# AIS-Bonn/stillleben

Measured on AMD Instinct MI355X. Metric: scenes/sec (settle + 640x480 6-ch GT render), 20-obj YCB-like, higher is better.
Workload: dtype f32; 1 GPU; C2: 20 of 21 procedural YCB-like objects (8k verts/16k tris, 1024^2 texture each) per scene; per step and GPU 32768 scenes are staged (random stack), settled (100 frames x 4 substeps), framed (camera, light, shadow matrix) and rendered at 640x480 (rgb, coord+depth, class, instance, normals; shadows on, SSAO on) -- all four stages inside the timed region; render_chunk=512, objects=20, settle_streams=1, render_streams=2, pair_contact_budget=0, parallelism=1 GPU

## Files before the change

include/slhip.h:

```cpp
#ifndef SLHIP_H
#define SLHIP_H

#include <stdint.h>

#ifdef __cplusplus
extern "C" {
#endif

#define SLHIP_ABI_VERSION 5
#define SLHIP_NUM_LIGHTS 3


typedef struct {
    float* d_env;
    float* d_irradiance;
    float* d_prefilter;
    float* d_brdf_lut;
    uint32_t env_size, env_levels;
    uint32_t irr_size;
    uint32_t pre_size, pre_levels;
    uint32_t lut_size;
} slhip_light_map;

typedef struct {
// ... 252 lines not shown
    uint32_t max_contacts_per_scene;
    uint32_t pair_contact_budget;
    uint32_t resume;
    uint32_t max_body_pairs_per_scene;
    float stabilization_threshold;
    uint32_t _pad_params;
} slhip_settle_params;
#define SLHIP_STAB_DAMPING          0.5f
#define SLHIP_STAB_GRAVITY          0.9f
#define SLHIP_STAB_FREEZE_INTERVAL  1.5f
#define SLHIP_STAB_FREEZE_TOLERANCE 0.25f
#define SLHIP_STAB_MAX_INTERACTIONS 10

#define SLHIP_MAX_BODIES     400
#define SLHIP_DEFAULT_HULL_PAIRS 2048
#define SLHIP_DEFAULT_CONTACTS   1024
#define SLHIP_PAIR_CACHE_DENSE_HULLS 256

int slhip_settle(const slhip_settle_scene* d_scenes, uint32_t n_scenes,
                 slhip_body* d_bodies, const slhip_hull* d_hulls, const float* d_hull_verts,
                 const slhip_settle_params* params, void* d_scratch, uint64_t scratch_bytes,
                 void* stream);
#define SLHIP_SETTLE_REFUSED_BODIES 1u
#define SLHIP_SETTLE_REFUSED_HULLS  2u
int slhip_settle_caps(const void* d_scratch, uint32_t n_scenes, const slhip_settle_params* params,
                      uint64_t counts[10], void* stream);
int slhip_settle_status(const void* d_scratch, uint32_t n_scenes, uint32_t* h_status, uint32_t* h_n_refused,
                        void* stream);
int slhip_settle_timing_enable(int on);
int slhip_settle_timings(float avg_ms_out[5], uint32_t launches_out[5]);
int slhip_settle_timing_every(uint32_t every);
int slhip_settle_timings_by_step(float* ms_out, uint32_t* steps_out, uint32_t capacity, uint32_t* n_out);
int slhip_settle_solver_wave_lds(void);
int slhip_settle_scratch_bytes(uint32_t n_scenes, const slhip_settle_params* params, uint64_t* bytes_out);

int slhip_overlap_any(const slhip_settle_scene* d_scenes, uint32_t n_scenes,
                      const slhip_body* d_bodies, const slhip_hull* d_hulls,
                      const float* d_hull_verts, uint8_t* d_flags, void* stream);


int slhip_diff_sobel_valid(const int16_t* d_inst, const float* d_depth, int depth_stride, int H, int W,
                           uint8_t* d_valid, void* stream);

int slhip_diff_dilate(const uint8_t* d_mask, const uint8_t* d_valid, const float* d_coords, int coord_stride,
                      int H, int W, uint8_t* d_out_mask, float* d_out_coords, void* stream);

int slhip_diff_image_gradients(const uint8_t* d_rgb, const uint8_t* d_valid, int H, int W, float* d_grad_x,
                               float* d_grad_y, void* stream);

int slhip_diff_pose_backward(const uint8_t* d_rgb, const float* d_coord, const int16_t* d_inst,
                             const float* d_grad_img, const float* h_proj, const float* d_poses,
                             const int32_t* d_obj_inst, int n_obj, int H, int W, uint8_t* d_valid,
                             double* d_acc, float* d_out, void* stream);
int slhip_diff_pose_backward_batch(const uint8_t* d_rgb, const float* d_coord, const int16_t* d_inst,
                                   const float* d_grad_img, uint64_t grad_stride_floats, const float* h_proj,
                                   const float* d_poses, const int32_t* d_obj_inst, int n_obj, int n_hyp, int H, int W,
                                   uint8_t* d_valid, double* d_acc, float* d_out, void* stream);

int slhip_light_map_floats(uint32_t env_size, uint32_t env_levels, uint32_t irr_size, uint32_t pre_size,
                           uint32_t pre_levels, uint32_t lut_size, uint64_t out[4]);
int slhip_light_map_build(const float* d_equirect, int H, int W, const slhip_light_map* lm, void* stream);

typedef struct {
    float translation[6];
    float scaling[3];
    float blur_kernel[25];
// ... 173 lines not shown
```

stillleben_amd/_abi.py:

```python
import ctypes as C
import os

import numpy as np

NUM_LIGHTS = 3
CHUNK_TRIS = 256

DRAW_HAS_BASE_TEX = 1
DRAW_VERTEX_COLORS = 2
DRAW_CASTS_SHADOW = 4
DRAW_ALPHA_TEST = 8
DRAW_NO_VERTEX_ID = 16
DRAW_HAS_NORMAL_TEX = 32
DRAW_HAS_MR_TEX = 64
DRAW_HAS_OCCLUSION_TEX = 128
DRAW_HAS_EMISSIVE_TEX = 256
DRAW_HAS_STICKER = 512
SAMPLER_DEFAULT = 0x10 | 0x20 | (2 << 6)

OUT_RGB = 0x01
OUT_COORD = 0x02
OUT_CLASS = 0x04
OUT_INSTANCE = 0x08
OUT_NORMALS = 0x10
# ... 276 lines not shown
    L.slhip_diff_sobel_valid.argtypes = [C.c_void_p, C.c_void_p, C.c_int, C.c_int, C.c_int, C.c_void_p, C.c_void_p]
    L.slhip_diff_dilate.argtypes = [C.c_void_p, C.c_void_p, C.c_void_p, C.c_int, C.c_int, C.c_int, C.c_void_p, C.c_void_p, C.c_void_p]
    L.slhip_diff_image_gradients.argtypes = [C.c_void_p, C.c_void_p, C.c_int, C.c_int, C.c_void_p, C.c_void_p, C.c_void_p]
    L.slhip_diff_pose_backward.argtypes = [C.c_void_p] * 7 + [C.c_int, C.c_int, C.c_int] + [C.c_void_p] * 4
    L.slhip_diff_pose_backward_batch.argtypes = [C.c_void_p] * 4 + [C.c_uint64] + [C.c_void_p] * 3 + [C.c_int] * 4 + [C.c_void_p] * 4
    L.slhip_diff_vertex_backward.argtypes = [C.c_void_p] * 8 + [C.c_int, C.c_int, C.c_int] + [C.c_void_p] * 4
    L.slhip_settle.argtypes = [C.c_void_p, C.c_uint32, C.c_void_p, C.c_void_p, C.c_void_p, C.c_void_p,
                               C.c_void_p, C.c_uint64, C.c_void_p]
    L.slhip_settle_status.argtypes = [C.c_void_p, C.c_uint32, C.c_void_p, C.POINTER(C.c_uint32), C.c_void_p]
    L.slhip_host_shadow_matrices.argtypes = [C.c_void_p, C.c_void_p, C.c_void_p]
    L.slhip_host_normal_matrix.argtypes = [C.c_void_p, C.c_void_p]
    L.slhip_host_convex_hull.argtypes = [C.c_void_p, C.c_uint32, C.c_void_p, C.c_uint32, C.POINTER(C.c_uint32)]
    L.slhip_host_fill_holes.argtypes = [C.c_void_p, C.c_uint32, C.c_uint32, C.c_uint32]
    L.slhip_records_count.argtypes = [C.c_void_p, C.c_uint32, C.c_void_p, C.c_void_p, C.POINTER(C.c_uint32), C.POINTER(C.c_uint32)]
    L.slhip_records_build_render.argtypes = [C.c_void_p, C.c_uint32, C.c_void_p, C.c_void_p, C.c_uint32, C.c_void_p, C.c_void_p,
                                             C.c_uint32, C.c_void_p, C.c_uint32]
    L.slhip_render_object_stats.argtypes = [
        C.POINTER(MeshPool), C.c_void_p, C.c_void_p, C.c_void_p, C.c_uint32, C.c_uint32, C.c_uint32, C.c_uint32, C.c_uint32,
        C.POINTER(RenderScratch), C.c_uint32, C.c_void_p, C.c_uint64, C.c_void_p, C.POINTER(C.c_uint64), C.c_void_p,
    ]
    L.slhip_render_object_stats_bytes.argtypes = [C.c_uint32, C.c_uint32, C.c_uint32, C.c_uint32, C.POINTER(C.c_uint64)]
    L.slhip_render_object_masks.argtypes = [
        C.POINTER(MeshPool), C.c_void_p, C.c_void_p, C.c_void_p, C.c_uint32, C.c_uint32, C.c_uint32, C.c_uint32, C.c_uint32,
        C.POINTER(RenderScratch), C.c_uint32, C.c_void_p, C.c_uint64, C.c_void_p, C.POINTER(C.c_uint64),
        C.c_void_p, C.c_void_p, C.c_uint64, C.POINTER(C.c_uint64), C.c_void_p,
    ]
    L.slhip_render_object_masks_bytes.argtypes = [C.c_uint32, C.c_uint32, C.c_uint32, C.c_uint32, C.POINTER(C.c_uint64),
                                                  C.POINTER(C.c_uint64)]
    L.slhip_object_masks_expand.argtypes = [C.c_void_p, C.c_void_p, C.c_uint32, C.c_uint32, C.c_uint32, C.c_uint32, C.c_uint32,
                                            C.c_void_p, C.c_uint64, C.c_void_p, C.c_void_p]
    L.slhip_render_ssao_skipped.argtypes = [C.c_void_p, C.c_uint32, C.c_uint32, C.c_uint32, C.POINTER(C.c_uint64 * 2), C.c_void_p]
    L.slhip_render_ssao_levels.argtypes = [C.c_void_p, C.c_uint32, C.c_uint32, C.c_uint32, C.POINTER(C.c_uint64 * 8), C.c_void_p]
    L.slhip_render_ssao_level_tables.argtypes = [C.POINTER(C.c_float * 5), C.POINTER(C.c_uint32 * 6), C.POINTER(C.c_uint8 * 384)]
    L.slhip_settle_caps.argtypes = [C.c_void_p, C.c_uint32, C.c_void_p, C.POINTER(C.c_uint64 * 10), C.c_void_p]
    L.slhip_settle_timing_enable.argtypes = [C.c_int]
    L.slhip_settle_timings.argtypes = [C.POINTER(C.c_float * 5), C.POINTER(C.c_uint32 * 5)]
    if hasattr(L, "slhip_settle_timing_every"):
        L.slhip_settle_timing_every.argtypes = [C.c_uint32]
        L.slhip_settle_timings_by_step.argtypes = [C.c_void_p, C.c_void_p, C.c_uint32, C.POINTER(C.c_uint32)]
    L.slhip_settle_scratch_bytes.argtypes = [C.c_uint32, C.c_void_p, C.POINTER(C.c_uint64)]
    L.slhip_overlap_any.argtypes = [C.c_void_p, C.c_uint32, C.c_void_p, C.c_void_p, C.c_void_p, C.c_void_p, C.c_void_p]
    L.slhip_light_map_floats.argtypes = [C.c_uint32] * 6 + [C.POINTER(C.c_uint64 * 4)]
    L.slhip_light_map_build.argtypes = [C.c_void_p, C.c_int, C.c_int, C.c_void_p, C.c_void_p]
    L.slhip_camera_model.argtypes = [C.c_void_p, C.c_void_p, C.c_void_p, C.c_uint32, C.c_int, C.c_int, C.c_void_p, C.c_void_p]
    L.slhip_stream_create_cu_range.argtypes = [C.c_uint32, C.c_uint32, C.POINTER(C.c_void_p)]
    L.slhip_stream_destroy.argtypes = [C.c_void_p]
    L.slhip_synth_stage.argtypes = [C.c_void_p] * 8
    L.slhip_synth_place.argtypes = [C.c_void_p] * 10
    if hasattr(L, "slhip_synth_place_env"):
        L.slhip_synth_place_env.argtypes = [C.c_void_p, C.POINTER(SynthEnv)] + [C.c_void_p] * 10
    if hasattr(L, "slhip_synth_place_view"):
        L.slhip_synth_place_view.argtypes = [C.c_void_p, C.POINTER(SynthEnv), C.POINTER(SynthView)] + [C.c_void_p] * 10
    L.slhip_comm_unique_id.argtypes = [C.c_void_p]
    L.slhip_comm_create.argtypes = [C.c_void_p, C.c_int, C.c_int, C.POINTER(C.c_void_p)]
    L.slhip_comm_destroy.argtypes = [C.c_void_p]
    L.slhip_comm_info.argtypes = [C.c_void_p, C.POINTER(C.c_int), C.POINTER(C.c_int)]
    L.slhip_allgather.argtypes = [C.c_void_p, C.c_void_p, C.c_void_p, C.c_uint64, C.c_void_p]
    L.slhip_allgather_group.argtypes = [C.c_void_p, C.c_uint32, C.c_void_p, C.c_void_p, C.c_void_p, C.c_void_p]
    _LIB = L
    return L


def check(status, what):
    if status != 0:
        msg = lib().slhip_last_error()
        raise SlhipError("%s failed (%d): %s" % (what, status, msg.decode() if msg else "?"))
# ... 1 lines not shown
```

stillleben_amd/csrc/slhip_settle.hip:

```cpp
#include "slhip_common.h"
#include <vector>
#include <cstdlib>

namespace {

static_assert(sizeof(slhip_body) == 304, "slhip_body layout");
static_assert(sizeof(slhip_hull) == 64, "slhip_hull layout");
static_assert(sizeof(slhip_settle_params) == 128, "slhip_settle_params layout");

constexpr int kMaxContactsPerHP = 4;
constexpr float kInf = 3.0e38f;
constexpr float kDepthWeight = 30.0f;

struct v3 { float x, y, z; };
struct quat { float x, y, z, w; };
struct m3 { float m[9]; };

__device__ __forceinline__ v3 V(float x, float y, float z) { v3 r; r.x = x; r.y = y; r.z = z; return r; }
__device__ __forceinline__ v3 add(v3 a, v3 b) { return V(a.x + b.x, a.y + b.y, a.z + b.z); }
__device__ __forceinline__ v3 sub(v3 a, v3 b) { return V(a.x - b.x, a.y - b.y, a.z - b.z); }
__device__ __forceinline__ v3 scale(v3 a, float s) { return V(a.x * s, a.y * s, a.z * s); }
__device__ __forceinline__ v3 neg(v3 a) { return V(-a.x, -a.y, -a.z); }
__device__ __forceinline__ float dot(v3 a, v3 b) { return fmaf(a.z, b.z, fmaf(a.y, b.y, a.x * b.x)); }
__device__ __forceinline__ v3 cross(v3 a, v3 b)
{
    return V(a.y * b.z - a.z * b.y, a.z * b.x - a.x * b.z, a.x * b.y - a.y * b.x);
}
__device__ __forceinline__ v3 madd(v3 a, v3 b, float s)
{
    return V(fmaf(b.x, s, a.x), fmaf(b.y, s, a.y), fmaf(b.z, s, a.z));
}
__device__ __forceinline__ v3 m3_mul(const m3& M, v3 v)
{
// ... 1409 lines not shown
    for (auto& r : g_settle_timing.pending) {
        float ms = 0.0f;
        if (failed || hipEventSynchronize(r.e1) != hipSuccess || hipEventElapsedTime(&ms, r.e0, r.e1) != hipSuccess) { failed = true; continue; }
        acc[r.kernel] += ms;
        ++n[r.kernel];
        if (by_step_ms) {
            if (r.kernel == 0) {
                row_open = rows < cap;
                if (row_open) { if (steps_out) steps_out[rows] = r.step; ++rows; }
            }
            if (row_open) by_step_ms[5 * (size_t)(rows - 1) + r.kernel] = ms;
        }
    }
    for (hipEvent_t e : g_settle_timing.events) (void)hipEventDestroy(e);
    g_settle_timing.events.clear();
    g_settle_timing.pending.clear();
    if (n_out) *n_out = rows;
    if (failed) {
        slhip::set_error("slhip_settle_timings: event readback failed");
        return -1;
    }
    for (int k = 0; k < 5; ++k) {
        if (avg_ms_out) avg_ms_out[k] = n[k] ? (float)(acc[k] / n[k]) : 0.0f;
        if (launches_out) launches_out[k] = n[k];
    }
    return 0;
}

extern "C" int slhip_settle_timings(float avg_ms_out[5], uint32_t launches_out[5])
{
    return settle_timings_read(avg_ms_out, launches_out, nullptr, nullptr, 0, nullptr);
}

#ifdef SLHIP_ROW_PROFILE
extern "C" int slhip_settle_row_profile(unsigned long long out[8])
{
    SLHIP_CHECK(hipDeviceSynchronize());
    SLHIP_CHECK(hipMemcpyFromSymbol(out, HIP_SYMBOL(g_row_prof), 8 * sizeof(unsigned long long)));
    unsigned long long zero[8] = {0, 0, 0, 0, 0, 0, 0, 0};
    SLHIP_CHECK(hipMemcpyToSymbol(HIP_SYMBOL(g_row_prof), zero, sizeof(zero)));
    return 0;
}
#endif

static int g_last_solve_lds = 0;
extern "C" int slhip_settle_solver_wave_lds(void) { return g_last_solve_lds; }

extern "C" int slhip_settle_timing_every(uint32_t every)
{
    g_settle_timing_every = every ? every : 1u;
    return 0;
}

extern "C" int slhip_settle_timings_by_step(float* ms_out, uint32_t* steps_out, uint32_t capacity, uint32_t* n_out)
{
    if (!ms_out || !n_out) {
        slhip::set_error("slhip_settle_timings_by_step: null output");
        return -1;
    }
    return settle_timings_read(nullptr, nullptr, ms_out, steps_out, capacity, n_out);
}

extern "C" int slhip_settle_scratch_bytes(uint32_t n_scenes, const slhip_settle_params* params, uint64_t* bytes_out)
{
    if (!bytes_out) {
        slhip::set_error("slhip_settle_scratch_bytes: null output");
        return -1;
    }
    *bytes_out = settle_scratch_bytes(n_scenes, params);
    return 0;
}

extern "C" int slhip_settle(const slhip_settle_scene* d_scenes, uint32_t n_scenes, slhip_body* d_bodies,
                            const slhip_hull* d_hulls, const float* d_hull_verts, const slhip_settle_params* params,
                            void* d_scratch, uint64_t scratch_bytes, void* stream_)
{
// ... 8 lines not shown
        return -1;
    }
    const SettleDims D = settle_dims(params);
    const int nb_cap = D.nb_cap;
    if (nb_cap > SLHIP_MAX_BODIES) {
        slhip::set_error("slhip_settle: at most %d bodies per scene", SLHIP_MAX_BODIES);
        return -1;
    }
    {
        if (n_scenes > 65535u) {
            slhip::set_error("slhip_settle: at most 65535 scenes per launch");
            return -1;
        }
        ProfScratch* prof_w = reinterpret_cast<ProfScratch*>(d_scratch);
        DriveAcc* drive_w = reinterpret_cast<DriveAcc*>(prof_w + n_scenes);
        char* base = reinterpret_cast<char*>(d_scratch) + settle_fixed_bytes(n_scenes, D);
        PairCache pc;
        pc.base = reinterpret_cast<int4*>(base);
        pc.stride = D.cache_stride;
        pc.hashed = D.cache_hashed;
        WideBufs W = wide_carve(base + settle_cache_bytes(n_scenes, D), n_scenes, nb_cap, D.lh_cap, D.p_cap, D.c_cap, D.bp_cap);
        if (((uint64_t)n_scenes << W.pair_bits) > (1ull << 32)) {
            slhip::set_error("slhip_settle: n_scenes x max_hull_pairs_per_scene exceeds the 32-bit work list entries");
            return -1;
        }
        const BeginLds BL = begin_layout(nb_cap, D.lh_cap);
        const FinishLds FL = finish_layout(nb_cap, W.g_cap);
        int solve_lds = 20 * 1024;
        if (solve_min_lds(nb_cap, W.g_cap) > solve_lds) solve_lds = (solve_min_lds(nb_cap, W.g_cap) + 1023) & ~1023;
        if (const char* e = getenv("SLHIP_SOLVE_LDS_KB")) { const int kb = atoi(e) * 1024; if (kb >= solve_min_lds(nb_cap, W.g_cap) && kb <= 160 * 1024) solve_lds = kb; }
        int max_class = 2;
        if (const char* e = getenv("SLHIP_SOLVE_SPW")) { const int v = atoi(e); max_class = v == 1 ? 0 : v == 2 ? 1 : 2; }
        W.solve_lds = solve_lds; W.solve_max_class = max_class;
        g_last_solve_lds = solve_lds;
        if (BL.total > 160 * 1024 || FL.total > 160 * 1024 || solve_lds > 160 * 1024) {
            slhip::set_error("slhip_settle: scenes of %d bodies / %d hulls do not fit the kernels' LDS", nb_cap, D.lh_cap);
            return -1;
        }
        SLHIP_CHECK(hipFuncSetAttribute(reinterpret_cast<const void*>(k_w_begin), hipFuncAttributeMaxDynamicSharedMemorySize, BL.total));
        SLHIP_CHECK(hipFuncSetAttribute(reinterpret_cast<const void*>(k_w_finish), hipFuncAttributeMaxDynamicSharedMemorySize, FL.total));
        SLHIP_CHECK(hipFuncSetAttribute(reinterpret_cast<const void*>(k_w_solve), hipFuncAttributeMaxDynamicSharedMemorySize, solve_lds));
        if (params->resume == 0u) k_w_prologue<<<n_scenes, 64, 0, stream>>>(d_scenes, d_bodies, d_hulls, W, prof_w, pc);
        const unsigned list_stride = n_scenes * (unsigned)D.p_cap;
        unsigned work_grid = n_scenes < 16u ? n_scenes * 8u : n_scenes;
        if (const char* e = getenv("SLHIP_WORK_GRID_DIV")) { const unsigned d = (unsigned)atoi(e); if (d > 1u && work_grid / d >= 64u) work_grid /= d; }
        bool persistent = n_scenes <= kPersistentMaxScenes;
        if (const char* e = getenv("SLHIP_SETTLE_PERSISTENT")) persistent = atoi(e) != 0;
        if (persistent) {
            WideBufs Wp = W;
            Wp.solve_lds = max(solve_lds, 32 * 1024);
            const int lds = max(max(BL.total, FL.total), Wp.solve_lds);
            SLHIP_CHECK(hipFuncSetAttribute(reinterpret_cast<const void*>(k_w_persistent), hipFuncAttributeMaxDynamicSharedMemorySize, lds));
            unsigned grid = n_scenes < 4096u ? n_scenes : 4096u;
            if (const char* e = getenv("SLHIP_SETTLE_PERSISTENT_GRID")) { const unsigned g = (unsigned)atoi(e); if (g > 0u && g < grid) grid = g; }
            k_w_persistent<<<grid, 64, lds, stream>>>(d_scenes, d_bodies, d_hulls, d_hull_verts, *params, Wp, BL, FL, pc, drive_w, list_stride, n_scenes);
            SLHIP_LAUNCH_CHECK();
            return 0;
        }
        uint32_t lockstep_frames = params->frames;
        if (const char* e = getenv("SLHIP_SETTLE_SWITCH_FRAME")) { const int v = atoi(e); if (v >= 0 && (uint32_t)v < params->frames) lockstep_frames = (uint32_t)v; }
        uint32_t step = params->resume;
        for (uint32_t f = 0; f < lockstep_frames; ++f)
            for (uint32_t sub = 0; sub < params->substeps; ++sub, ++step) {
                constexpr size_t kMaxTimedEvents = 1u << 16;
                bool timed = g_settle_timing.on && step % g_settle_timing_every == 0u && g_settle_timing.events.size() < kMaxTimedEvents;
                hipEvent_t ev[6];
// ... 112 lines not shown
```

stillleben_amd/csrc/slhip_settle_wide.inc:

```

struct WideHdr {
    int n_hp, n_groups, n_plane_groups, n_active, n_active_before_pairs, ncol, status, n_hulls;
    int hp_overflow, hp_found;
    int g_overflow;
    int lds_need, lds_class;
};
struct PlanePM { int stamp, count, c_off, id[4], pad; };
static_assert(sizeof(PlanePM) == 32, "PlanePM layout");

__device__ __forceinline__ int cache_x(int seed_n, bool has, unsigned step) { return (seed_n & 3) | ((has ? 1 : 0) << 2) | (int)(step << 3); }
__device__ __forceinline__ int sv_pack(int idx) { return (idx & 0xff) | ((idx >> 16) << 8); }
__device__ __forceinline__ int sv_unpack(int c) { return (c & 0xff) | (((c >> 8) & 0xff) << 16); }

enum { kCapSpillSteps = 0, kCapContactDropSteps, kCapPairDropSteps, kCapMaxContacts, kCapMaxPairs, kCapReducedSteps, kCapGroupDropSteps, kCapContactSum, kCapWords = 8 };
constexpr unsigned short kCulled = 0xffff;

__device__ const float kNoImpulse[4] = {0.0f, 0.0f, 0.0f, 0.0f};

struct WideBufs {
    WideHdr* hdr;
    WBody* wb;
    HullRef* lh;
    int* body_lh;
    HullPair* hp;
    unsigned short* hp_off;
    unsigned short* hp_grp;
    MainResult* mr;
    StagePt* stage;
    Contact* ac;
    Group* groups;
    unsigned short* order;
    unsigned* lpt_count;
    unsigned short* lpt_table;
    unsigned* work;
    PM* pm;
    float* lnout;
    PlanePM* pp;
    unsigned* caps;
    unsigned* work_count;
    int nb_cap, lh_cap;
    int p_cap, c_cap;
    int g_cap, o_stride;
    int pair_bits;
    int solve_lds;
    int solve_max_class;
};
constexpr int kLptWords = 3 * 256 + 3 * 8;

__host__ __device__ inline size_t wide_align(size_t x) { return (x + 255u) & ~(size_t)255u; }

__host__ __device__ inline int wide_g_cap(int nb_cap, int p_cap, int bp_cap)
{
    long long pairs = (long long)nb_cap * (nb_cap - 1) / 2;
    if (pairs > p_cap) pairs = p_cap;
    const long long lim = bp_cap > 0 ? (long long)bp_cap : 12ll * nb_cap + 64;
    if (pairs > lim) pairs = lim;
    return nb_cap + (int)pairs;
}

inline uint64_t wide_bytes(uint32_t n, int nb_cap, int lh_cap, int p_cap, int c_cap, int bp_cap)
{
    const size_t g_cap = (size_t)wide_g_cap(nb_cap, p_cap, bp_cap), o_stride = 2 * g_cap + 66;
    uint64_t b = 0;
    b += wide_align((size_t)n * sizeof(WideHdr));
    b += wide_align((size_t)n * nb_cap * sizeof(WBody));
    b += wide_align((size_t)n * lh_cap * sizeof(HullRef));
    b += wide_align((size_t)n * (nb_cap + 1) * sizeof(int));
    b += wide_align((size_t)n * p_cap * sizeof(HullPair));
    b += wide_align((size_t)n * (p_cap + 1) * sizeof(unsigned short));
    b += wide_align((size_t)n * p_cap * sizeof(unsigned short));
    b += wide_align((size_t)n * p_cap * sizeof(MainResult));
    b += wide_align((size_t)n * p_cap * 4 * sizeof(StagePt));
    b += wide_align((size_t)n * c_cap * sizeof(Contact));
    b += wide_align((size_t)n * g_cap * sizeof(Group));
    b += wide_align((size_t)n * o_stride * sizeof(unsigned short));
    b += wide_align((size_t)5 * n * p_cap * sizeof(unsigned));
    b += wide_align((size_t)2 * n * p_cap * sizeof(PM));
    b += wide_align((size_t)n * c_cap * sizeof(float));
// ... 4 lines not shown
    b += wide_align((size_t)3 * 256 * ((n + 7u) / 8u) * sizeof(unsigned short));
    return b;
}

inline WideBufs wide_carve(char* base, uint32_t n, int nb_cap, int lh_cap, int p_cap, int c_cap, int bp_cap)
{
    WideBufs B;
    B.nb_cap = nb_cap; B.lh_cap = lh_cap; B.p_cap = p_cap; B.c_cap = c_cap;
    B.g_cap = wide_g_cap(nb_cap, p_cap, bp_cap); B.o_stride = 2 * B.g_cap + 66;
    B.pair_bits = 1;
    while ((1 << B.pair_bits) < p_cap) ++B.pair_bits;
    char* p = base;
    auto take = [&](size_t bytes) { char* r = p; p += wide_align(bytes); return r; };
    B.hdr = reinterpret_cast<WideHdr*>(take((size_t)n * sizeof(WideHdr)));
    B.wb = reinterpret_cast<WBody*>(take((size_t)n * nb_cap * sizeof(WBody)));
    B.lh = reinterpret_cast<HullRef*>(take((size_t)n * lh_cap * sizeof(HullRef)));
    B.body_lh = reinterpret_cast<int*>(take((size_t)n * (nb_cap + 1) * sizeof(int)));
    B.hp = reinterpret_cast<HullPair*>(take((size_t)n * p_cap * sizeof(HullPair)));
    B.hp_off = reinterpret_cast<unsigned short*>(take((size_t)n * (p_cap + 1) * sizeof(unsigned short)));
    B.hp_grp = reinterpret_cast<unsigned short*>(take((size_t)n * p_cap * sizeof(unsigned short)));
    B.mr = reinterpret_cast<MainResult*>(take((size_t)n * p_cap * sizeof(MainResult)));
    B.stage = reinterpret_cast<StagePt*>(take((size_t)n * p_cap * 4 * sizeof(StagePt)));
    B.ac = reinterpret_cast<Contact*>(take((size_t)n * c_cap * sizeof(Contact)));
    B.groups = reinterpret_cast<Group*>(take((size_t)n * B.g_cap * sizeof(Group)));
    B.order = reinterpret_cast<unsigned short*>(take((size_t)n * B.o_stride * sizeof(unsigned short)));
    B.work = reinterpret_cast<unsigned*>(take((size_t)5 * n * p_cap * sizeof(unsigned)));
    B.pm = reinterpret_cast<PM*>(take((size_t)2 * n * p_cap * sizeof(PM)));
    B.lnout = reinterpret_cast<float*>(take((size_t)n * c_cap * sizeof(float)));
    B.pp = reinterpret_cast<PlanePM*>(take((size_t)n * nb_cap * sizeof(PlanePM)));
    B.caps = reinterpret_cast<unsigned*>(take((size_t)n * kCapWords * sizeof(unsigned)));
    B.work_count = reinterpret_cast<unsigned*>(take(64));
    B.lpt_count = reinterpret_cast<unsigned*>(take(kLptWords * sizeof(unsigned)));
    B.lpt_table = reinterpret_cast<unsigned short*>(take((size_t)3 * 256 * ((n + 7u) / 8u) * sizeof(unsigned short)));
    B.solve_lds = 0; B.solve_max_class = 2;
    return B;
}

struct PairCache {
    int4* base;
    unsigned stride;
    int hashed;
};
__device__ __forceinline__ int4* pair_cache_slot(const PairCache& pc, int s, int n_hulls, int la, int lb, unsigned parity, bool claim)
{
    int4* tab = pc.base + (size_t)s * pc.stride;
    if (!pc.hashed) {
        if (n_hulls <= 0 || (unsigned)n_hulls * (unsigned)n_hulls > pc.stride) return nullptr;
        return tab + (size_t)la * n_hulls + lb;
    }
    const unsigned half = pc.stride >> 1, mask = half - 1u;
    tab += (size_t)(parity & 1u) * half;
    const unsigned key = ((unsigned)la | ((unsigned)lb << 16)) + 1u;
    unsigned h = (key * 2654435761u) >> 7;
    for (unsigned probe = 0; probe < half; ++probe, ++h) {
        int4* e = tab + (h & mask);
        unsigned k = (unsigned)e->w;
        if (k == 0u) {
            if (!claim) return nullptr;
            k = atomicCAS(reinterpret_cast<unsigned*>(&e->w), 0u, key);
            if (k == 0u) k = key;
        }
        if (k == key) return e;
    }
    return nullptr;
}

__device__ __forceinline__ void lanes_copy(void* dst, const void* src, int bytes, int hl, int n_lanes)
// ... 59 lines not shown
        if (lane == 0) { prof_all[s].status = SLHIP_SETTLE_REFUSED_HULLS; H->status = 1; }
        return;
    }
    if (lane == 0) {
        body_lh[nb] = n_lh;
        prof_all[s].status = 0;
        H->status = 0;
        H->n_hp = 0; H->n_groups = 0; H->n_plane_groups = 0; H->n_active = 0; H->n_active_before_pairs = 0; H->ncol = 0;
        H->n_hulls = n_lh;
    }
    {
        const unsigned n = pc.hashed ? pc.stride : (unsigned)(n_lh * n_lh);
        if (n <= pc.stride) {
            int4* z = pc.base + (size_t)s * pc.stride;
            for (unsigned k = lane; k < n; k += 64) z[k] = make_int4(0, 0, 0, 0);
        }
    }
}

struct BeginLds { int off_wb, off_lh, off_body_lh, off_band, off_plist, total; };
__host__ __device__ inline BeginLds begin_layout(int nb_cap, int lh_cap)
{
    BeginLds L;
    int o = 0;
    auto take = [&](int bytes) { const int r = o; o += (bytes + 15) & ~15; return r; };
    L.off_wb = take(nb_cap * (int)sizeof(WBody));
    L.off_lh = take(lh_cap * (int)sizeof(HullRef));
    L.off_body_lh = take((nb_cap + 1) * 4);
    L.off_band = take(4 * kBandCap * (int)sizeof(BandPt));
    L.off_plist = take(64);
    L.total = o;
    return L;
}

template <bool kFileWork>
__device__ __forceinline__ void begin_scene(char* smem, const int s, const unsigned n_scenes, const slhip_settle_scene* __restrict__ scenes,
                                            slhip_body* bodies_all, const slhip_hull* __restrict__ hulls, const float* __restrict__ hull_verts,
                                            const slhip_settle_params& prm, const WideBufs& W, const BeginLds& L, DriveAcc* drive_all, unsigned step)
{
    const int lane = threadIdx.x;
    WideHdr* H = W.hdr + s;
    if (H->status != 0) return;
    WBody* wb = reinterpret_cast<WBody*>(smem + L.off_wb);
    HullRef* lh = reinterpret_cast<HullRef*>(smem + L.off_lh);
    int* body_lh = reinterpret_cast<int*>(smem + L.off_body_lh);
    BandPt* band = reinterpret_cast<BandPt*>(smem + L.off_band);
    unsigned char* plist = reinterpret_cast<unsigned char*>(smem + L.off_plist);
    const float4* gv = reinterpret_cast<const float4*>(hull_verts);
    const f3* hv = reinterpret_cast<const f3*>(hull_verts);
    const slhip_settle_scene sc = scenes[s];
    slhip_body* bodies = bodies_all + sc.body_begin;
    const int nb = (int)(sc.body_end - sc.body_begin);
    const float dt = prm.dt;
    DriveAcc* drv = drive_all + (size_t)s * W.nb_cap;
    Contact* ac = W.ac + (size_t)s * W.c_cap;
    Group* groups = W.groups + (size_t)s * W.g_cap;
    HullPair* hp = W.hp + (size_t)s * W.p_cap;
    const int c_cap = W.c_cap, p_cap = W.p_cap;

    for (int k = lane; k <= nb; k += 64) body_lh[k] = W.body_lh[(size_t)s * (W.nb_cap + 1) + k];
    __syncthreads();
    wave_copy_words(lh, W.lh + (size_t)s * W.lh_cap, body_lh[nb] * (int)sizeof(HullRef), lane);
    for (int i = lane; i < nb; i += 64) {
        load_body(bodies[i], wb[i]);
        update_world_inertia(bodies[i], wb[i]);
        if (wb[i].dynamic) {
            wb[i].v = madd(wb[i].v, V(prm.gravity[0], prm.gravity[1], prm.gravity[2]), dt * (1.0f - bodies[i].stab[1]));
            float damp = 1.0f - prm.angular_damping * dt;
            if (damp < 0.0f) damp = 0.0f;
            wb[i].w = scale(wb[i].w, damp);
        }
        if (bodies[i].drive_flags & 1u) {
            DriveAcc z;
            z.dl[0] = z.dl[1] = z.dl[2] = z.da[0] = z.da[1] = z.da[2] = 0.0f;
            drv[i] = z;
        }
    }
    __syncthreads();

    int n_groups = 0, n_active = 0;
    if (sc.has_plane) {
        int off_run = n_active;
        for (int base = 0; base < nb; base += 64) {
            const int i = base + lane;
            bool pass = false;
            if (i < nb && wb[i].dynamic) {
                const v3 ci = add(m3_mul(wb[i].R, V(bodies[i].bsphere[0], bodies[i].bsphere[1], bodies[i].bsphere[2])), wb[i].t);
                const float vz = wb[i].v.z < 0.0f ? -wb[i].v.z * dt : 0.0f;
                pass = !(ci.z - bodies[i].bsphere[3] - sc.plane_z > prm.contact_offset + vz);
            }
            const int rank = compact_slot(pass, 0);
            const int n_pass = __popcll(__ballot(pass));
            if (pass) plist[rank] = (unsigned char)lane;
            __syncthreads();
            const int sg = lane >> 4, sl = lane & 15;
            for (int r0 = 0; r0 < n_pass; r0 += 4) {
                const bool on = r0 + sg < n_pass;
                const int bi = on ? base + (int)plist[r0 + sg] : 0;
                RawContacts rc;
                rc.count = 0;
                int ids[4] = {0, 0, 0, 0};
                if (on) {
                    const float vz = wb[bi].v.z < 0.0f ? -wb[bi].v.z * dt : 0.0f;
                    plane_contacts_sg16(wb[bi], lh, hv, gv, body_lh[bi], body_lh[bi + 1], sc.plane_z,
                                        prm.contact_offset + vz, band + sg * kBandCap, sg, sl, rc, ids);
                }
                const int lead = rc.count >= 3 ? 1 : 0;
                const int rows = rc.count + lead;
                const int c0 = __shfl(rows, 0, 64), c1 = __shfl(rows, 16, 64), c2 = __shfl(rows, 32, 64);
                const int c3 = __shfl(rows, 48, 64);
                const int off = off_run + (sg > 0 ? c0 : 0) + (sg > 1 ? c1 : 0) + (sg > 2 ? c2 : 0);
// ... 16 lines not shown
                    if (sl < rc.count && off + lead + sl < c_cap) {
                        const float e = 0.5f * (bodies[bi].restitution + prm.plane_restitution);
                        const v3 pa = vsel(sl == 0, rc.pa[0], vsel(sl == 1, rc.pa[1], vsel(sl == 2, rc.pa[2], rc.pa[3])));
                        const float sp = sl == 0 ? rc.sep[0] : sl == 1 ? rc.sep[1] : sl == 2 ? rc.sep[2] : rc.sep[3];
                        float warm = 0.0f;
                        const float* lp = W.lnout + (size_t)s * c_cap + pc_off;
                        if (0 < pcount && q0.w == my_id) warm = kWarmStart * lp[0];
                        if (1 < pcount && q1.x == my_id) warm = kWarmStart * lp[1];
                        if (2 < pcount && q1.y == my_id) warm = kWarmStart * lp[2];
                        if (3 < pcount && q1.z == my_id) warm = kWarmStart * lp[3];
                        fill_contact(&ac[off + lead + sl], bi, -1, wb[bi], nullptr, pa, V(pa.x, pa.y, sc.plane_z), rc.n, sp,
                                     prm.rest_offset, e, sl == 0 && !lead, warm);
                    }
                    if (sl == 0) {
                        Group G;
                        G.a = (unsigned short)bi; G.b = (unsigned short)kNoBody;
                        G.begin = (unsigned short)min(off, c_cap); G.end = (unsigned short)min(off + rows, c_cap);
                        G.color = 0;
                        groups[n_groups + r0 + sg] = G;
                        const int written = max(0, min(rc.count, c_cap - off - lead));
                        reinterpret_cast<int4*>(ppm)[0] = make_int4((int)step, written, off + lead, ids[0]);
                        reinterpret_cast<int4*>(ppm)[1] = make_int4(ids[1], ids[2], ids[3], (lead && off < c_cap) ? 1 : 0);
                    }
                }
                off_run += c0 + c1 + c2 + c3;
                __syncthreads();
            }
            n_groups += n_pass;
        }
        n_active = off_run;
    }
    const int n_plane_groups = n_groups;

    int n_hp = 0, hp_found = 0, g_overflow = 0;
    {
        const int n_pairs = nb * (nb - 1) / 2;
        for (int base = 0; base < n_pairs; base += 64) {
            const int p = base + lane;
            bool pass = false;
            int pi = 0, pj = 0;
            if (p < n_pairs) {
                int rem = p, row = nb - 1;
                while (rem >= row) { rem -= row; ++pi; --row; }
                pj = pi + 1 + rem;
                if (wb[pi].dynamic || wb[pj].dynamic) {
                    const v3 ci = add(m3_mul(wb[pi].R, V(bodies[pi].bsphere[0], bodies[pi].bsphere[1], bodies[pi].bsphere[2])), wb[pi].t);
                    const v3 cj = add(m3_mul(wb[pj].R, V(bodies[pj].bsphere[0], bodies[pj].bsphere[1], bodies[pj].bsphere[2])), wb[pj].t);
                    const v3 dv = sub(wb[pi].v, wb[pj].v);
                    const float margin = 2.0f * prm.contact_offset + sqrtf(dot(dv, dv)) * dt;
                    const v3 d = sub(ci, cj);
                    const float rr = bodies[pi].bsphere[3] + bodies[pj].bsphere[3] + margin;
                    pass = !(dot(d, d) > rr * rr);
                }
            }
            unsigned long long mask = __ballot(pass);
            while (mask) {
                const int src = __ffsll((long long)mask) - 1;
                mask &= mask - 1;
                const int i = __shfl(pi, src, 64), j = __shfl(pj, src, 64);
                const int la0 = body_lh[i], na = body_lh[i + 1] - la0;
                const int lb0 = body_lh[j], nbh = body_lh[j + 1] - lb0;
                const unsigned ga0 = bodies[i].hull_begin, gb0 = bodies[j].hull_begin;
                const v3 dv = sub(wb[i].v, wb[j].v);
                const float margin = 2.0f * prm.contact_offset + sqrtf(dot(dv, dv)) * dt;
                const int first = n_hp;
                const int combos = na * nbh;
                for (int cb = 0; cb < combos; cb += 64) {
                    const int q = cb + lane;
                    bool ok = false;
                    int a = 0, b = 0;
                    if (q < combos) {
                        a = q / nbh; b = q % nbh;
                        const HullRef& A = lh[la0 + a];
                        const HullRef& B = lh[lb0 + b];
                        const v3 ca = add(m3_mul(wb[i].R, A.sc), wb[i].t);
                        const v3 cbw = add(m3_mul(wb[j].R, B.sc), wb[j].t);
                        const v3 dd = sub(ca, cbw);
                        const float r2 = A.sr + B.sr + margin;
                        ok = !(dot(dd, dd) > r2 * r2);
                        if (ok) ok = aabb_overlap(wb[i], hulls[ga0 + a], wb[j], hulls[gb0 + b], margin);
                    }
                    const int slot = compact_slot(ok, n_hp);
                    if (ok && slot < p_cap) hp[slot] = hp_pack(i, j, a, b);
                    const int n_ok = (int)__popcll(__ballot(ok));
                    hp_found += n_ok;
                    n_hp = min(n_hp + n_ok, p_cap);
                }
                if (n_hp > first && n_groups >= W.g_cap) {
                    g_overflow = 1;
                    n_hp = first;
                }
                if (n_hp > first) {
                    if (lane == 0) {
                        Group G;
                        G.a = (unsigned short)i; G.b = (unsigned short)j;
                        G.begin = 0; G.end = 0;
                        G.color = 0;
                        groups[n_groups] = G;
                    }
                    ++n_groups;
                }
            }
        }
    }
    __syncthreads();
    wave_copy_words(W.wb + (size_t)s * W.nb_cap, wb, nb * (int)sizeof(WBody), lane);
    if (kFileWork && n_hp > 0) {
        const size_t region = (size_t)n_scenes * p_cap;
        int cnt0 = 0, cnt1 = 0, cnt2 = 0;
        for (int k0 = 0; k0 < n_hp; k0 += 64) {
            const int k = k0 + lane;
            int cls = -1;
            if (k < n_hp) {
                const HullPair e = hp[k];
                const int m = max(lh[body_lh[hp_ba(e)] + hp_ha(e)].count, lh[body_lh[hp_bb(e)] + hp_hb(e)].count);
                cls = m <= 16 ? 0 : m <= 32 ? 1 : 2;
            }
            cnt0 += (int)__popcll(__ballot(cls == 0)); cnt1 += (int)__popcll(__ballot(cls == 1)); cnt2 += (int)__popcll(__ballot(cls == 2));
        }
        unsigned base = 0u;
        if (lane < 3) {
            const int c = lane == 0 ? cnt0 : lane == 1 ? cnt1 : cnt2;
            if (c > 0) base = atomicAdd(&W.work_count[8 + lane], (unsigned)c);
        }
        unsigned run0 = (unsigned)__shfl((int)base, 0, 64), run1 = (unsigned)__shfl((int)base, 1, 64), run2 = (unsigned)__shfl((int)base, 2, 64);
        for (int k0 = 0; k0 < n_hp; k0 += 64) {
            const int k = k0 + lane;
            int cls = -1;
            if (k < n_hp) {
                const HullPair e = hp[k];
                const int m = max(lh[body_lh[hp_ba(e)] + hp_ha(e)].count, lh[body_lh[hp_bb(e)] + hp_hb(e)].count);
                cls = m <= 16 ? 0 : m <= 32 ? 1 : 2;
            }
            const unsigned long long m0 = __ballot(cls == 0), m1 = __ballot(cls == 1), m2 = __ballot(cls == 2);
            const unsigned long long below = (1ull << lane) - 1ull;
            const unsigned entry = ((unsigned)s << W.pair_bits) | (unsigned)k;
            if (cls == 0) W.work[run0 + (unsigned)__popcll(m0 & below)] = entry;
            if (cls == 1) W.work[region + run1 + (unsigned)__popcll(m1 & below)] = entry;
            if (cls == 2) W.work[2 * region + run2 + (unsigned)__popcll(m2 & below)] = entry;
            run0 += (unsigned)__popcll(m0); run1 += (unsigned)__popcll(m1); run2 += (unsigned)__popcll(m2);
        }
    }
    if (lane == 0) {
        H->n_hp = n_hp; H->n_groups = n_groups; H->n_plane_groups = n_plane_groups;
        H->n_active_before_pairs = n_active; H->n_active = n_active;
        H->hp_overflow = hp_found > p_cap ? 1 : 0; H->hp_found = hp_found; H->g_overflow = g_overflow;
    }
}

__global__ __launch_bounds__(64) __attribute__((amdgpu_waves_per_eu(5))) void k_w_begin(const slhip_settle_scene* __restrict__ scenes, slhip_body* bodies_all,
                                               const slhip_hull* __restrict__ hulls, const float* __restrict__ hull_verts,
                                               slhip_settle_params prm, WideBufs W, BeginLds L, DriveAcc* drive_all, unsigned step)
{
    extern __shared__ __attribute__((aligned(16))) char smem[];
    if (blockIdx.x == 0) for (int k = threadIdx.x; k < kLptWords; k += 64) W.lpt_count[k] = 0u;
    begin_scene<true>(smem, (int)blockIdx.x, gridDim.x, scenes, bodies_all, hulls, hull_verts, prm, W, L, drive_all, step);
}

__device__ __forceinline__ int gjk_work_item(unsigned e_work, const float* __restrict__ hull_verts, const slhip_settle_params& prm,
                                              const WideBufs& W, const PairCache& pc, int max_iter,
                                              unsigned step, unsigned n_scenes, bool& unfinished)
{
    const int s = (int)(e_work >> W.pair_bits), k = (int)(e_work & ((1u << W.pair_bits) - 1u));
    WideHdr* H = W.hdr + s;
    const float4* gv = reinterpret_cast<const float4*>(hull_verts);
    const WBody* wb = W.wb + (size_t)s * W.nb_cap;
    const HullRef* lh = W.lh + (size_t)s * W.lh_cap;
    const int* body_lh = W.body_lh + (size_t)s * (W.nb_cap + 1);
    MainResult mr;
    mr.type = 0; mr.dist = 0.0f;
    mr.n = V(0, 0, 0); mr.pa = V(0, 0, 0); mr.pb = V(0, 0, 0);
    mr.seed.n = 0; mr.seed.i0 = mr.seed.i1 = mr.seed.i2 = 0;
    const HullPair e = W.hp[(size_t)s * W.p_cap + k];
    const int ba = hp_ba(e), bb = hp_bb(e);
    const WBody wa = wb[ba], wbb = wb[bb];
    const v3 dv = sub(wa.v, wbb.v);
    const float margin = 2.0f * prm.contact_offset + sqrtf(dot(dv, dv)) * prm.dt;
    const int la = body_lh[ba] + hp_ha(e), lb = body_lh[bb] + hp_hb(e);
    GjkSeed cached;
    cached.n = 0; cached.i0 = cached.i1 = cached.i2 = 0;
// ... 1261 lines not shown
```

Before: 10180 scenes/s.

## Flatten broad-phase hull-pair tests across all near body pairs per wave batch

```diff
diff --git a/include/slhip.h b/include/slhip.h
--- a/include/slhip.h
+++ b/include/slhip.h
@@ -308,6 +308,7 @@
 int slhip_settle_timing_every(uint32_t every);
 int slhip_settle_timings_by_step(float* ms_out, uint32_t* steps_out, uint32_t capacity, uint32_t* n_out);
 int slhip_settle_solver_wave_lds(void);
+int slhip_settle_pair_decode_table(uint32_t nb, uint16_t* ij);
 int slhip_settle_scratch_bytes(uint32_t n_scenes, const slhip_settle_params* params, uint64_t* bytes_out);
 
 int slhip_overlap_any(const slhip_settle_scene* d_scenes, uint32_t n_scenes,
diff --git a/stillleben_amd/_abi.py b/stillleben_amd/_abi.py
--- a/stillleben_amd/_abi.py
+++ b/stillleben_amd/_abi.py
@@ -332,6 +332,8 @@
     L.slhip_render_ssao_skipped.argtypes = [C.c_void_p, C.c_uint32, C.c_uint32, C.c_uint32, C.POINTER(C.c_uint64 * 2), C.c_void_p]
     L.slhip_render_ssao_levels.argtypes = [C.c_void_p, C.c_uint32, C.c_uint32, C.c_uint32, C.POINTER(C.c_uint64 * 8), C.c_void_p]
     L.slhip_render_ssao_level_tables.argtypes = [C.POINTER(C.c_float * 5), C.POINTER(C.c_uint32 * 6), C.POINTER(C.c_uint8 * 384)]
+    if hasattr(L, "slhip_settle_pair_decode_table"):
+        L.slhip_settle_pair_decode_table.argtypes = [C.c_uint32, C.c_void_p]
     L.slhip_settle_caps.argtypes = [C.c_void_p, C.c_uint32, C.c_void_p, C.POINTER(C.c_uint64 * 10), C.c_void_p]
     L.slhip_settle_timing_enable.argtypes = [C.c_int]
     L.slhip_settle_timings.argtypes = [C.POINTER(C.c_float * 5), C.POINTER(C.c_uint32 * 5)]
diff --git a/stillleben_amd/csrc/slhip_pair_decode.h b/stillleben_amd/csrc/slhip_pair_decode.h
--- /dev/null
+++ b/stillleben_amd/csrc/slhip_pair_decode.h
@@ -0,0 +1,22 @@
+#pragma once
+#include <math.h>
+
+#if defined(__HIPCC__) || defined(__CUDACC__)
+#define SLHIP_HD __host__ __device__
+#else
+#define SLHIP_HD
+#endif
+
+SLHIP_HD inline int slhip_pair_row_start(int i, int nb) { return i * (2 * nb - 1 - i) / 2; }
+
+SLHIP_HD inline void slhip_pair_decode(int p, int nb, int* pi, int* pj)
+{
+    const int m = 2 * nb - 1;
+    int i = (int)(((float)m - sqrtf((float)(m * m - 8 * p))) * 0.5f);
+    if (i < 0) i = 0;
+    if (i > nb - 2) i = nb - 2;
+    while (slhip_pair_row_start(i, nb) > p) --i;
+    while (slhip_pair_row_start(i + 1, nb) <= p) ++i;
+    *pi = i;
+    *pj = i + 1 + (p - slhip_pair_row_start(i, nb));
+}
diff --git a/stillleben_amd/csrc/slhip_settle.hip b/stillleben_amd/csrc/slhip_settle.hip
--- a/stillleben_amd/csrc/slhip_settle.hip
+++ b/stillleben_amd/csrc/slhip_settle.hip
@@ -1,4 +1,5 @@
 #include "slhip_common.h"
+#include "slhip_pair_decode.h"
 #include <vector>
 #include <cstdlib>
 
@@ -1474,6 +1475,17 @@
     return settle_timings_read(avg_ms_out, launches_out, nullptr, nullptr, 0, nullptr);
 }
 
+#ifdef SLHIP_BEGIN_PROFILE
+extern "C" int slhip_settle_begin_profile(unsigned long long out[16])
+{
+    SLHIP_CHECK(hipDeviceSynchronize());
+    SLHIP_CHECK(hipMemcpyFromSymbol(out, HIP_SYMBOL(g_begin_prof), 16 * sizeof(unsigned long long)));
+    unsigned long long zero[16] = {0};
+    SLHIP_CHECK(hipMemcpyToSymbol(HIP_SYMBOL(g_begin_prof), zero, sizeof(zero)));
+    return 0;
+}
+#endif
+
 #ifdef SLHIP_ROW_PROFILE
 extern "C" int slhip_settle_row_profile(unsigned long long out[8])
 {
@@ -1484,6 +1496,21 @@
     return 0;
 }
 #endif
+
+extern "C" int slhip_settle_pair_decode_table(uint32_t nb, uint16_t* ij)
+{
+    if (!ij || nb > (uint32_t)SLHIP_MAX_BODIES) {
+        slhip::set_error("slhip_settle_pair_decode_table: null output or more than %d bodies", SLHIP_MAX_BODIES);
+        return -1;
+    }
+    const int n = (int)nb, n_pairs = n * (n - 1) / 2;
+    for (int p = 0; p < n_pairs; ++p) {
+        int i, j;
+        slhip_pair_decode(p, n, &i, &j);
+        ij[2 * p] = (uint16_t)i; ij[2 * p + 1] = (uint16_t)j;
+    }
+    return 0;
+}
 
 static int g_last_solve_lds = 0;
 extern "C" int slhip_settle_solver_wave_lds(void) { return g_last_solve_lds; }
@@ -1558,6 +1585,7 @@
         int max_class = 2;
         if (const char* e = getenv("SLHIP_SOLVE_SPW")) { const int v = atoi(e); max_class = v == 1 ? 0 : v == 2 ? 1 : 2; }
         W.solve_lds = solve_lds; W.solve_max_class = max_class;
+        if (const char* e = getenv("SLHIP_BEGIN_FLAT")) W.begin_flat = atoi(e) != 0 ? 1 : 0;
         g_last_solve_lds = solve_lds;
         if (BL.total > 160 * 1024 || FL.total > 160 * 1024 || solve_lds > 160 * 1024) {
             slhip::set_error("slhip_settle: scenes of %d bodies / %d hulls do not fit the kernels' LDS", nb_cap, D.lh_cap);
diff --git a/stillleben_amd/csrc/slhip_settle_wide.inc b/stillleben_amd/csrc/slhip_settle_wide.inc
--- a/stillleben_amd/csrc/slhip_settle_wide.inc
+++ b/stillleben_amd/csrc/slhip_settle_wide.inc
@@ -44,6 +44,7 @@
     int pair_bits;
     int solve_lds;
     int solve_max_class;
+    int begin_flat;
 };
 constexpr int kLptWords = 3 * 256 + 3 * 8;
 
@@ -114,7 +115,7 @@
     B.work_count = reinterpret_cast<unsigned*>(take(64));
     B.lpt_count = reinterpret_cast<unsigned*>(take(kLptWords * sizeof(unsigned)));
     B.lpt_table = reinterpret_cast<unsigned short*>(take((size_t)3 * 256 * ((n + 7u) / 8u) * sizeof(unsigned short)));
-    B.solve_lds = 0; B.solve_max_class = 2;
+    B.solve_lds = 0; B.solve_max_class = 2; B.begin_flat = 1;
     return B;
 }
 
@@ -240,6 +241,25 @@
     L.total = o;
     return L;
 }
+
+constexpr int kPackedPairs = 64;
+static_assert(kPackedPairs * (2 * (int)sizeof(int4) + (int)sizeof(int)) <= 4 * kBandCap * (int)sizeof(BandPt), "the packed pairs fit the band cache");
+
+#ifdef SLHIP_BEGIN_PROFILE
+__device__ unsigned long long g_begin_prof[16];
+__device__ __forceinline__ unsigned long long begp_now()
+{
+    asm volatile("s_waitcnt vmcnt(0) lgkmcnt(0)" ::: "memory");
+    return __builtin_amdgcn_s_memtime();
+}
+#define BEGP(...) __VA_ARGS__
+#define BEGP_ADD(slot_, val_) do { if ((threadIdx.x & 63u) == 0u) atomicAdd(&g_begin_prof[slot_], (unsigned long long)(val_)); } while (0)
+#else
+#define BEGP(...)
+#define BEGP_ADD(slot_, val_)
+#endif
+
+struct BpState { int n_hp, hp_found, n_groups, g_overflow, cnt1, cnt2; };
 
 template <bool kFileWork>
 __device__ __forceinline__ void begin_scene(char* smem, const int s, const unsigned n_scenes, const slhip_settle_scene* __restrict__ scenes,
@@ -265,6 +285,7 @@
     Group* groups = W.groups + (size_t)s * W.g_cap;
     HullPair* hp = W.hp + (size_t)s * W.p_cap;
     const int c_cap = W.c_cap, p_cap = W.p_cap;
+    BEGP(const unsigned long long t_a = begp_now();)
 
     for (int k = lane; k <= nb; k += 64) body_lh[k] = W.body_lh[(size_t)s * (W.nb_cap + 1) + k];
     __syncthreads();
@@ -285,6 +306,7 @@
         }
     }
     __syncthreads();
+    BEGP(const unsigned long long t_b = begp_now();)
 
     int n_groups = 0, n_active = 0;
     if (sc.has_plane) {
@@ -367,95 +389,187 @@
     }
     const int n_plane_groups = n_groups;
 
-    int n_hp = 0, hp_found = 0, g_overflow = 0;
+    BEGP(const unsigned long long t_c = begp_now(); unsigned long long bp_c1 = 0ull, bp_c2 = 0ull;
+         unsigned bp_passes = 0u, bp_combos = 0u, bp_pairs = 0u, bp_batches = 0u, bp_again = 0u;)
+    BpState st;
+    st.n_hp = 0; st.hp_found = 0; st.n_groups = n_groups; st.g_overflow = 0; st.cnt1 = 0; st.cnt2 = 0;
     {
+        int4* pk = reinterpret_cast<int4*>(smem + L.off_band);
+        int* hits = reinterpret_cast<int*>(pk + 2 * kPackedPairs);
+        const unsigned long long below = (1ull << lane) - 1ull;
         const int n_pairs = nb * (nb - 1) / 2;
         for (int base = 0; base < n_pairs; base += 64) {
+            BEGP(const unsigned long long t0 = begp_now();)
             const int p = base + lane;
             bool pass = false;
             int pi = 0, pj = 0;
+            float margin_l = 0.0f;
             if (p < n_pairs) {
-                int rem = p, row = nb - 1;
-                while (rem >= row) { rem -= row; ++pi; --row; }
-                pj = pi + 1 + rem;
+                slhip_pair_decode(p, nb, &pi, &pj);
                 if (wb[pi].dynamic || wb[pj].dynamic) {
                     const v3 ci = add(m3_mul(wb[pi].R, V(bodies[pi].bsphere[0], bodies[pi].bsphere[1], bodies[pi].bsphere[2])), wb[pi].t);
                     const v3 cj = add(m3_mul(wb[pj].R, V(bodies[pj].bsphere[0], bodies[pj].bsphere[1], bodies[pj].bsphere[2])), wb[pj].t);
                     const v3 dv = sub(wb[pi].v, wb[pj].v);
-                    const float margin = 2.0f * prm.contact_offset + sqrtf(dot(dv, dv)) * dt;
+                    margin_l = 2.0f * prm.contact_offset + sqrtf(dot(dv, dv)) * dt;
                     const v3 d = sub(ci, cj);
-                    const float rr = bodies[pi].bsphere[3] + bodies[pj].bsphere[3] + margin;
+                    const float rr = bodies[pi].bsphere[3] + bodies[pj].bsphere[3] + margin_l;
                     pass = !(dot(d, d) > rr * rr);
                 }
             }
             unsigned long long mask = __ballot(pass);
-            while (mask) {
-                const int src = __ffsll((long long)mask) - 1;
-                mask &= mask - 1;
-                const int i = __shfl(pi, src, 64), j = __shfl(pj, src, 64);
-                const int la0 = body_lh[i], na = body_lh[i + 1] - la0;
-                const int lb0 = body_lh[j], nbh = body_lh[j + 1] - lb0;
-                const unsigned ga0 = bodies[i].hull_begin, gb0 = bodies[j].hull_begin;
-                const v3 dv = sub(wb[i].v, wb[j].v);
-                const float margin = 2.0f * prm.contact_offset + sqrtf(dot(dv, dv)) * dt;
-                const int first = n_hp;
-                const int combos = na * nbh;
-                for (int cb = 0; cb < combos; cb += 64) {
-                    const int q = cb + lane;
-                    bool ok = false;
-                    int a = 0, b = 0;
-                    if (q < combos) {
-                        a = q / nbh; b = q % nbh;
-                        const HullRef& A = lh[la0 + a];
-                        const HullRef& B = lh[lb0 + b];
-                        const v3 ca = add(m3_mul(wb[i].R, A.sc), wb[i].t);
-                        const v3 cbw = add(m3_mul(wb[j].R, B.sc), wb[j].t);
-                        const v3 dd = sub(ca, cbw);
-                        const float r2 = A.sr + B.sr + margin;
-                        ok = !(dot(dd, dd) > r2 * r2);
-                        if (ok) ok = aabb_overlap(wb[i], hulls[ga0 + a], wb[j], hulls[gb0 + b], margin);
+            BEGP(const unsigned long long t1 = begp_now(); bp_c1 += t1 - t0;)
+            if (mask == 0ull) continue;
+            BEGP(bp_pairs += (unsigned)__popcll(mask); ++bp_batches;)
+            const BpState st0 = st;
+            bool serial = W.begin_flat == 0;
+            if (!serial) {
+                const int rank = __popcll(mask & below), n_near = __popcll(mask);
+                int la0 = 0, lb0 = 0, nbh = 0, combos = 0;
+                if (pass) {
+                    la0 = body_lh[pi]; lb0 = body_lh[pj];
+                    nbh = body_lh[pj + 1] - lb0;
+                    combos = (body_lh[pi + 1] - la0) * nbh;
+                }
+                serial = __ballot(combos > (1 << 24)) != 0ull;
+                if (!serial) {
+                    int total;
+                    const int start = wave_excl_scan(combos, total);
+                    if (pass) {
+                        pk[2 * rank] = make_int4(pi | (pj << 16), la0, lb0, nbh);
+                        pk[2 * rank + 1] = make_int4((int)bodies[pi].hull_begin, (int)bodies[pj].hull_begin, __float_as_int(margin_l), start);
                     }
-                    const int slot = compact_slot(ok, n_hp);
-                    if (ok && slot < p_cap) hp[slot] = hp_pack(i, j, a, b);
-                    const int n_ok = (int)__popcll(__ballot(ok));
-                    hp_found += n_ok;
-                    n_hp = min(n_hp + n_ok, p_cap);
+                    hits[lane] = 0;
+                    __syncthreads();
+                    for (int f0 = 0; f0 < total; f0 += 64) {
+                        const int f = f0 + lane;
+                        bool ok = false;
+                        int r = 0, i = 0, j = 0, a = 0, b = 0, big = 0;
+                        if (f < total) {
+#pragma unroll
+                            for (int half = 32; half > 0; half >>= 1) {
+                                const int t = r + half;
+                                if (t < n_near && pk[2 * t + 1].w <= f) r = t;
+                            }
+                            const int4 c0 = pk[2 * r], c1 = pk[2 * r + 1];
+                            i = c0.x & 0xffff; j = (int)((unsigned)c0.x >> 16);
+                            const int q = f - c1.w;
+                            if (c0.w == 1) a = q;
+                            else { a = q / c0.w; b = q % c0.w; }
+                            const float margin = __int_as_float(c1.z);
+                            const HullRef& A = lh[c0.y + a];
+                            const HullRef& B = lh[c0.z + b];
+                            const v3 ca = add(m3_mul(wb[i].R, A.sc), wb[i].t);
+                            const v3 cbw = add(m3_mul(wb[j].R, B.sc), wb[j].t);
+                            const v3 dd = sub(ca, cbw);
+                            const float r2 = A.sr + B.sr + margin;
+                            ok = !(dot(dd, dd) > r2 * r2);
+                            if (ok) ok = aabb_overlap(wb[i], hulls[(unsigned)c1.x + (unsigned)a], wb[j], hulls[(unsigned)c1.y + (unsigned)b], margin);
+                            big = max(A.count, B.count);
+                        }
+                        const int slot = compact_slot(ok, st.n_hp);
+                        const bool listed = ok && slot < p_cap;
+                        if (listed) hp[slot] = hp_pack(i, j, a, b);
+                        if (ok) atomicAdd(&hits[r], 1);
+                        const int n_ok = (int)__popcll(__ballot(ok));
+                        st.hp_found += n_ok;
+                        st.n_hp = min(st.n_hp + n_ok, p_cap);
+                        if (kFileWork) {
+                            st.cnt1 += (int)__popcll(__ballot(listed && big > 16 && big <= 32));
+                            st.cnt2 += (int)__popcll(__ballot(listed && big > 32));
+                        }
+                        BEGP(++bp_passes; bp_combos += (unsigned)min(64, total - f0);)
+                    }
+                    __syncthreads();
+                    const bool hit = pass && hits[rank] > 0;
+                    const unsigned long long hm = __ballot(hit);
+                    const int n_hit = __popcll(hm);
+                    if (st.hp_found - st0.hp_found > p_cap - st0.n_hp || st0.n_groups + n_hit > W.g_cap) {
+                        st = st0;
+                        serial = true;
+                        BEGP(++bp_again;)
+                    } else {
+                        if (hit) {
+                            Group G;
+                            G.a = (unsigned short)pi; G.b = (unsigned short)pj;
+                            G.begin = 0; G.end = 0;
+                            G.color = 0;
+                            groups[st.n_groups + __popcll(hm & below)] = G;
+                        }
+                        st.n_groups += n_hit;
+                    }
                 }
-                if (n_hp > first && n_groups >= W.g_cap) {
-                    g_overflow = 1;
-                    n_hp = first;
+            }
+            if (serial) {
+                while (mask) {
+                    const int src = __ffsll((long long)mask) - 1;
+                    mask &= mask - 1;
+                    const int i = __shfl(pi, src, 64), j = __shfl(pj, src, 64);
+                    const int la0 = body_lh[i], na = body_lh[i + 1] - la0;
+                    const int lb0 = body_lh[j], nbh = body_lh[j + 1] - lb0;
+                    const unsigned ga0 = bodies[i].hull_begin, gb0 = bodies[j].hull_begin;
+                    const v3 dv = sub(wb[i].v, wb[j].v);
+                    const float margin = 2.0f * prm.contact_offset + sqrtf(dot(dv, dv)) * dt;
+                    const BpState first = st;
+                    const int combos = na * nbh;
+                    for (int cb = 0; cb < combos; cb += 64) {
+                        const int q = cb + lane;
+                        bool ok = false;
+                        int a = 0, b = 0, big = 0;
+                        if (q < combos) {
+                            a = q / nbh; b = q % nbh;
+                            const HullRef& A = lh[la0 + a];
+                            const HullRef& B = lh[lb0 + b];
+                            const v3 ca = add(m3_mul(wb[i].R, A.sc), wb[i].t);
+                            const v3 cbw = add(m3_mul(wb[j].R, B.sc), wb[j].t);
+                            const v3 dd = sub(ca, cbw);
+                            const float r2 = A.sr + B.sr + margin;
+                            ok = !(dot(dd, dd) > r2 * r2);
+                            if (ok) ok = aabb_overlap(wb[i], hulls[ga0 + a], wb[j], hulls[gb0 + b], margin);
+                            big = max(A.count, B.count);
+                        }
+                        const int slot = compact_slot(ok, st.n_hp);
+                        const bool listed = ok && slot < p_cap;
+                        if (listed) hp[slot] = hp_pack(i, j, a, b);
+                        const int n_ok = (int)__popcll(__ballot(ok));
+                        st.hp_found += n_ok;
+                        st.n_hp = min(st.n_hp + n_ok, p_cap);
+                        if (kFileWork) {
+                            st.cnt1 += (int)__popcll(__ballot(listed && big > 16 && big <= 32));
+                            st.cnt2 += (int)__popcll(__ballot(listed && big > 32));
+                        }
+                        BEGP(++bp_passes; bp_combos += (unsigned)min(64, combos - cb);)
+                    }
+                    if (st.n_hp > first.n_hp && st.n_groups >= W.g_cap) {
+                        st.g_overflow = 1;
+                        st.n_hp = first.n_hp; st.cnt1 = first.cnt1; st.cnt2 = first.cnt2;
+                    }
+                    if (st.n_hp > first.n_hp) {
+                        if (lane == 0) {
+                            Group G;
+                            G.a = (unsigned short)i; G.b = (unsigned short)j;
+                            G.begin = 0; G.end = 0;
+                            G.color = 0;
+                            groups[st.n_groups] = G;
+                        }
+                        ++st.n_groups;
+                    }
                 }
-                if (n_hp > first) {
-                    if (lane == 0) {
-                        Group G;
-                        G.a = (unsigned short)i; G.b = (unsigned short)j;
-                        G.begin = 0; G.end = 0;
-                        G.color = 0;
-                        groups[n_groups] = G;
-                    }
-                    ++n_groups;
-                }
-            }
-        }
-    }
+            }
+            BEGP(bp_c2 += begp_now() - t1;)
+        }
+    }
+    const int n_hp = st.n_hp, hp_found = st.hp_found, g_overflow = st.g_overflow;
+    n_groups = st.n_groups;
     __syncthreads();
+    BEGP(const unsigned long long t_copy = begp_now();)
     wave_copy_words(W.wb + (size_t)s * W.nb_cap, wb, nb * (int)sizeof(WBody), lane);
+    BEGP(const unsigned long long t_file = begp_now();)
     if (kFileWork && n_hp > 0) {
         const size_t region = (size_t)n_scenes * p_cap;
-        int cnt0 = 0, cnt1 = 0, cnt2 = 0;
-        for (int k0 = 0; k0 < n_hp; k0 += 64) {
-            const int k = k0 + lane;
-            int cls = -1;
-            if (k < n_hp) {
-                const HullPair e = hp[k];
-                const int m = max(lh[body_lh[hp_ba(e)] + hp_ha(e)].count, lh[body_lh[hp_bb(e)] + hp_hb(e)].count);
-                cls = m <= 16 ? 0 : m <= 32 ? 1 : 2;
-            }
-            cnt0 += (int)__popcll(__ballot(cls == 0)); cnt1 += (int)__popcll(__ballot(cls == 1)); cnt2 += (int)__popcll(__ballot(cls == 2));
-        }
+        const unsigned long long below = (1ull << lane) - 1ull;
         unsigned base = 0u;
         if (lane < 3) {
-            const int c = lane == 0 ? cnt0 : lane == 1 ? cnt1 : cnt2;
+            const int c = lane == 0 ? n_hp - st.cnt1 - st.cnt2 : lane == 1 ? st.cnt1 : st.cnt2;
             if (c > 0) base = atomicAdd(&W.work_count[8 + lane], (unsigned)c);
         }
         unsigned run0 = (unsigned)__shfl((int)base, 0, 64), run1 = (unsigned)__shfl((int)base, 1, 64), run2 = (unsigned)__shfl((int)base, 2, 64);
@@ -468,7 +582,6 @@
                 cls = m <= 16 ? 0 : m <= 32 ? 1 : 2;
             }
             const unsigned long long m0 = __ballot(cls == 0), m1 = __ballot(cls == 1), m2 = __ballot(cls == 2);
-            const unsigned long long below = (1ull << lane) - 1ull;
             const unsigned entry = ((unsigned)s << W.pair_bits) | (unsigned)k;
             if (cls == 0) W.work[run0 + (unsigned)__popcll(m0 & below)] = entry;
             if (cls == 1) W.work[region + run1 + (unsigned)__popcll(m1 & below)] = entry;
@@ -481,6 +594,10 @@
         H->n_active_before_pairs = n_active; H->n_active = n_active;
         H->hp_overflow = hp_found > p_cap ? 1 : 0; H->hp_found = hp_found; H->g_overflow = g_overflow;
     }
+    BEGP(const unsigned long long t_end = begp_now();
+         BEGP_ADD(0, 1); BEGP_ADD(1, t_b - t_a); BEGP_ADD(2, t_c - t_b); BEGP_ADD(3, bp_c1); BEGP_ADD(4, bp_c2);
+         BEGP_ADD(5, t_file - t_copy); BEGP_ADD(6, t_end - t_file); BEGP_ADD(7, t_end - t_a);
+         BEGP_ADD(8, bp_passes); BEGP_ADD(9, bp_combos); BEGP_ADD(10, bp_pairs); BEGP_ADD(11, bp_batches); BEGP_ADD(12, bp_again);)
 }
 
 __global__ __launch_bounds__(64) __attribute__((amdgpu_waves_per_eu(5))) void k_w_begin(const slhip_settle_scene* __restrict__ scenes, slhip_body* bodies_all,
```

New measurement: 10210 scenes/s, median of 4. No clear change (+0.3%).
